# ligengen/EgoGen

Hardware: AMD Instinct MI355X
Metric: PPO env-steps/sec (512 parallel SMPL-X agents) (higher is better)
Workload: dtype f32 (blend GEMM: shape/template columns as 2-term bf16 splits, pose correctives as one fp16 product, fp32 accumulate); PPO update products on 2-term bf16 splits; rollout policy layers on 2-term bf16 splits

## Files before the change

### egogen_amd/_lib.py

```python
from __future__ import annotations

import ctypes as C
import os

_HERE = os.path.dirname(os.path.abspath(__file__))
LIB_PATH = os.path.join(_HERE, "libegogen_hip.so")

c_float_p = C.POINTER(C.c_float)
c_int_p = C.POINTER(C.c_int32)


class EgxError(RuntimeError):
    pass


class BodyModelHost(C.Structure):
    _fields_ = [
        ("num_verts", C.c_int),
        ("v_template_host", C.c_void_p), ("shapedirs_host", C.c_void_p), ("posedirs_host", C.c_void_p),
        ("J_regressor_host", C.c_void_p), ("parents_host", C.c_void_p), ("lbs_weights_host", C.c_void_p),
        ("hand_comps_l_host", C.c_void_p), ("hand_comps_r_host", C.c_void_p),
        ("hand_mean_l_host", C.c_void_p), ("hand_mean_r_host", C.c_void_p),
        ("extra_vids_host", C.c_void_p), ("lmk_vids_host", C.c_void_p), ("lmk_bary_host", C.c_void_p),
        ("num_markers", C.c_int), ("marker_vids_host", C.c_void_p),
# ... 143 lines not shown
    "egx_sample_action": (C.c_int, [C.c_void_p, C.c_void_p, C.c_void_p, C.c_float, C.c_float, C.c_int, C.c_int, C.c_void_p,
                                    C.c_void_p, C.c_void_p]),
    "egx_gae": (C.c_int, [C.c_void_p, C.c_void_p, C.c_void_p, C.c_int, C.c_int, C.c_double, C.c_double, C.c_void_p,
                          C.c_void_p, C.c_void_p]),
    "egx_ppo_loss": (C.c_int, [C.c_void_p] * 9 + [C.c_float] * 6 + [C.c_int] + [C.c_void_p] * 5),
    "egx_gru_pointwise_bwd": (C.c_int, [C.c_void_p, C.c_void_p, C.c_void_p, C.c_void_p, C.c_int, C.c_int, C.c_void_p, C.c_void_p,
                                        C.c_void_p, C.c_void_p]),
    "egx_ppo_loss_packed": (C.c_int, [C.c_void_p] * 8 + [C.c_float] * 6 + [C.c_int] + [C.c_void_p] * 4),
    "egx_lbs_set_blend_mode": (C.c_int, [C.c_int]),
    "egx_lbs_get_blend_mode": (C.c_int, []),
    "egx_lbs_set_wave_tile": (C.c_int, [C.c_int]),
    "egx_lbs_get_wave_tile": (C.c_int, []),
    "egx_lbs_set_fix_queue_capacity": (C.c_int, [C.c_int]),
    "egx_lbs_fix_stats": (C.c_int, [C.c_void_p, C.c_void_p, C.c_int, C.POINTER(C.c_int32)]),
    "egx_gather_rows": (C.c_int, [C.c_void_p, C.c_int, C.c_int, C.c_void_p, C.c_void_p, C.c_void_p, C.c_void_p]),
    "egx_adv_stats": (C.c_int, [C.c_void_p, C.c_int, C.c_void_p, C.c_void_p]),
    "egx_track_episode": (C.c_int, [C.c_void_p, C.c_void_p, C.c_int, C.c_void_p, C.c_void_p, C.c_void_p, C.c_void_p]),
    "egx_rollout_store": (C.c_int, [C.c_void_p] * 6 + [C.c_int] + [C.c_void_p] * 10),
    "egx_adamw_workspace_floats": (C.c_size_t, []),
    "egx_adamw_clip_step": (C.c_int, [C.c_void_p, C.c_void_p, C.c_void_p, C.c_void_p, C.c_size_t, C.c_size_t, C.c_float] + [C.c_double] * 5 +
                            [C.c_void_p, C.c_void_p, C.c_void_p]),
    "egx_policy_set_precision": (C.c_int, [C.c_int]),
    "egx_policy_get_precision": (C.c_int, []),
    "egx_act_fwd": (C.c_int, [C.c_void_p, C.c_void_p, C.c_void_p, C.c_int, C.c_int, C.c_int, C.c_float, C.c_void_p]),
    "egx_act_bwd_colsum": (C.c_int, [C.c_void_p, C.c_void_p, C.c_void_p, C.c_void_p, C.c_int, C.c_int, C.c_int, C.c_float,
                                     C.c_void_p]),
    "egx_profile_next_lbs": (C.c_int, [C.c_void_p, C.c_void_p]),
    "egx_event_create": (C.c_int, [C.POINTER(C.c_void_p)]),
    "egx_event_destroy": (C.c_int, [C.c_void_p]),
    "egx_event_elapsed_ms": (C.c_int, [C.c_void_p, C.c_void_p, C.POINTER(C.c_float)]),
    "egx_policy_train_create": (C.c_int, [C.POINTER(PolicyWeights), C.POINTER(PolicyGrads), C.c_int, C.POINTER(C.c_void_p)]),
    "egx_policy_train_destroy": (None, [C.c_void_p]),
    "egx_policy_train_refresh": (C.c_int, [C.c_void_p, C.c_void_p]),
    "egx_policy_train_packed": (C.c_int, [C.c_void_p, C.POINTER(PolicyPacked3)]),
    "egx_policy_train_bind": (C.c_int, [C.c_void_p, C.c_void_p, C.c_void_p]),
    "egx_policy_train_step": (C.c_int, [C.c_void_p] * 9 + [C.c_float] * 6 + [C.c_void_p, C.c_void_p]),
    "egx_policy_train_step_heads": (C.c_int, [C.c_void_p] * 9 + [C.c_float] * 6 + [C.c_void_p, C.c_void_p]),
    "egx_policy_train_step_encoders": (C.c_int, [C.c_void_p, C.c_void_p]),
    "egx_policy_train_set_precision": (C.c_int, [C.c_void_p, C.c_int]),
    "egx_pack3_bytes": (C.c_size_t, [C.c_int, C.c_int]),
    "egx_pack3": (C.c_int, [C.c_void_p, C.c_int, C.c_int, C.c_int, C.c_int, C.c_void_p, C.c_int, C.c_int, C.c_void_p]),
    "egx_gemm3_workspace_bytes": (C.c_size_t, [C.c_int, C.c_int, C.c_int]),
    "egx_gemm3": (C.c_int, [C.c_void_p, C.c_int, C.c_int, C.c_void_p, C.c_int, C.c_int, C.c_int, C.c_int, C.c_int, C.c_void_p, C.c_int,
                            C.c_float, C.c_void_p, C.c_int, C.c_void_p, C.c_int, C.c_void_p, C.c_int, C.c_void_p, C.c_size_t, C.c_void_p]),
    "egx_vposer_workspace_bytes": (C.c_size_t, [C.c_int]),
    "egx_vposer_encode": (C.c_int, [C.POINTER(VposerWeights), C.c_void_p, C.c_int, C.c_int, C.c_void_p, C.c_void_p,
                                    C.c_size_t, C.c_void_p]),
}

_lib = None


def load():
    global _lib
    if _lib is not None:
        return _lib
    if not os.path.exists(LIB_PATH):
        raise EgxError(f"{LIB_PATH} not found - build it with `python -c 'import __graft_entry__ as g; g.build()'` "
                       f"or `make -C egogen_amd/csrc`; there is no CPU fallback")
    lib = C.CDLL(LIB_PATH)
    for name, (res, args) in SIGNATURES.items():
        fn = getattr(lib, name)
        fn.restype = res
        fn.argtypes = args
    _lib = lib
    return lib


def check(rc: int, what: str):
    if rc != 0:
        msg = load().egx_last_error()
        raise EgxError(f"{what} failed (code {rc}): {msg.decode() if msg else ''}")


def ptr(t):
    if t is None:
        return None
    assert t.is_contiguous(), "tensor must be contiguous"
    return C.c_void_p(t.data_ptr())


def current_stream_ptr():
    import torch
    return C.c_void_p(torch.cuda.current_stream().cuda_stream)
```

### egogen_amd/csrc/egx_nets.h

```cpp
#pragma once
#include "egx_common.h"

struct EgxSeg {
  const float* p;
  int w, ld;
};

int egx_launch_linear(hipStream_t st, int M, int N, const EgxSeg* segs, int nseg, const float* W, const float* b,
                      int act, float slope, const float* res, int ldr, float* out, int ldo);
int egx_launch_gru_pointwise(hipStream_t st, const float* gi, const float* gh, const float* hprev, int ldh, float* hout,
                             int ldo, int M, int H);
int egx_launch_cont6d_to_aa(hipStream_t st, const float* xb6, int n, float* out, int ldo);
int egx_launch_posenc(hipStream_t st, const float* dist, const float* time, int A, float* out);

void egx_launch_frame_scan(hipStream_t st, float* y, const float* x_last, int x_ld, int A, int width, int T);

struct D3Pack {
  const float* src;
  int R, K, ld, col0;
  void* dst;
  int S_total, s0;
  int transpose = 0;
};
void egx_launch_pack3(hipStream_t st, const D3Pack* jobs, int njobs);
// ... 4 lines not shown
  const bf16x8* B = nullptr;
  int S = 0;
  const float* bias = nullptr;
  const float* res = nullptr;
  int ldr = 0;
  float* out = nullptr;
  int ldo = 0;
  bf16x8* out3 = nullptr;
  int S3 = 0, s30 = 0;
  int M = 0, N = 0, act = 0;
  float slope = 0.f;
  int batches = 1;
  size_t batch_strideA = 0, batch_stride3 = 0;
  int batch_rows_out = 0;
  int prec = 0;
  float* out_act = nullptr;
  int ldact = 0;
  const float* dact = nullptr;
  int lddact = 0, dact_code = 0;
  float dact_slope = 0.f;
  bf16x8* out3T = nullptr;
  int S3T = 0, s3T0 = 0;
  float* bias_out = nullptr;
  int n_split = 0;
};
void egx_launch_dense3_n(hipStream_t st, const D3Plain* ps, int n);
void egx_launch_dense3(hipStream_t st, const D3Plain& p);
void egx_launch_dense3_pair(hipStream_t st, const D3Plain& p, const D3Plain& q);
void egx_launch_dense3_triple(hipStream_t st, const D3Plain& p, const D3Plain& q, const D3Plain& r);
int egx_ppo_loss_packed_precleared(const float* zp, const float* value, const float* act, const float* adv, const float* ret,
                                   const float* logp_old, const float* adv_stats, const float* scale, float adv_eps, float min_logvar,
                                   float max_logvar, float eps_clip, float vf_coef, float ent_coef, int num_rows, float* g_zp,
                                   float* g_value, float* out_terms, void* stream_);
void egx_launch_posenc3(hipStream_t st, const float* dist, const float* time, int n, float* out, int ld, void* out3, int S3, int s0,
                        void* out3T = nullptr, int S3T = 0, int col0T = 0, float* zero6 = nullptr );

struct D3Gru {
  const bf16x8* Ai = nullptr;
  int SAi = 0, sai0 = 0;
  const bf16x8* Bi = nullptr;
  int Si = 0;
  const float* bias_i = nullptr;
  const float* gi_in = nullptr;
  float* gi_out = nullptr;
  const bf16x8* Ah = nullptr;
  int SAh = 0, sah0 = 0;
  const bf16x8* Bh = nullptr;
  int Sh = 0;
  const float* bias_h = nullptr;
  const float* h_prev = nullptr;
  int ldh = 0;
  float* h_out = nullptr;
  int ldo = 0;
  bf16x8* h_out3 = nullptr;
  int S3 = 0, s30 = 0;
  int M = 0, H = 0;
  int prec = 0;
  float* gh_out = nullptr;
  bf16x8* h_out3T = nullptr;
  int S3T = 0, s3T0 = 0, col0T = 0;
};
int egx_launch_gru3(hipStream_t st, const D3Gru& g);
int egx_launch_gru3_pair(hipStream_t st, const D3Gru& g0, const D3Gru& g1);

struct RegWeights3 {
  const bf16x8 *in_m, *in_xb, *in_b3;
// ... 36 lines not shown
```

### egogen_amd/csrc/ppo.hip

```cpp
#include <algorithm>
#include <cstring>
#include "egx_common.h"

namespace {
constexpr float LOG_SQRT_2PI = 0.91893853320467274178f;

}

__device__ __forceinline__ float egx_wave_sum(float v) {
#pragma unroll
  for (int o = 32; o > 0; o >>= 1) v += __shfl_xor(v, o);
  return v;
}

__global__ __launch_bounds__(256) void egx_ppo_loss_kernel(const float* __restrict__ mu, const float* __restrict__ logvar,
                                                          const float* __restrict__ value, const float* __restrict__ act,
                                                          const float* __restrict__ adv, const float* __restrict__ ret,
                                                          const float* __restrict__ logp_old, const float* __restrict__ adv_stats,
                                                          const float* __restrict__ scale_ptr, float adv_eps, float min_lv,
                                                          float max_lv, float eps_clip, float vf_coef, float ent_coef, int n,
                                                          int stride ,
                                                          float* __restrict__ g_mu, float* __restrict__ g_logvar,
                                                          float* __restrict__ g_value, float* __restrict__ out_terms) {
  __shared__ float sh[4][6];
// ... 438 lines not shown
}

extern "C" int egx_rollout_store(const float* state, const float* egosensing, const float* dist, const float* time, const float* rew,
                                 const int32_t* term, int num_agents, float* state_dst, float* ego_dst, float* dist_dst, float* time_dst,
                                 float* rew_dst, int32_t* term_dst, float* ep_ret, float* ep_len, float* done_sums, void* stream_) {
  EGX_REQUIRE(state && egosensing && dist && time && state_dst && ego_dst && dist_dst && time_dst && num_agents > 0, "bad arguments");
  EGX_REQUIRE((!rew_dst && !term_dst && !ep_ret) || (rew && term && rew_dst && term_dst), "reward / termination source or slot missing");
  EGX_REQUIRE(!ep_ret || (ep_len && done_sums && rew && term), "episode bookkeeping needs ep_len, done_sums, rew, term");
  hipLaunchKernelGGL(egx_rollout_store_kernel, dim3(num_agents + (ep_ret ? 1 : 0)), dim3(256), 0, static_cast<hipStream_t>(stream_), state,
                     egosensing, dist, time, rew, term, num_agents, state_dst, ego_dst, dist_dst, time_dst, rew_dst, term_dst, ep_ret, ep_len,
                     done_sums);
  EGX_HIP_CHECK(hipGetLastError());
  return EGX_OK;
}

extern "C" size_t egx_adamw_workspace_floats(void) { return 1024 + 8; }

extern "C" int egx_adamw_clip_step(float* param, const float* grad, float* exp_avg, float* exp_avg_sq, size_t n, size_t n_clip,
                                   float max_norm, double lr, double beta1, double beta2, double eps, double weight_decay,
                                   float* step, float* workspace, void* stream_) {
  EGX_REQUIRE(param && grad && exp_avg && exp_avg_sq && step && workspace && n > 0 && n_clip <= n, "bad arguments");
  hipStream_t st = static_cast<hipStream_t>(stream_);
  const int nb = 1024;
  const bool do_clip = max_norm > 0.f && n_clip > 0;
  hipLaunchKernelGGL(egx_sumsq_partial_kernel, dim3(nb), dim3(256), 0, st, grad, do_clip ? n_clip : (size_t)0, workspace, step);
  hipLaunchKernelGGL(egx_adamw_consts_kernel, dim3(1), dim3(256), 0, st, workspace, nb, do_clip ? 1 : 0, max_norm, lr, beta1, beta2,
                     step, workspace + nb);
  const size_t blocks = (n + 1023) / 1024;
  hipLaunchKernelGGL(egx_adamw_flat_kernel, dim3((unsigned)blocks), dim3(256), 0, st, param, grad, exp_avg, exp_avg_sq, n, n_clip,
                     workspace + nb, lr, beta1, beta2, eps, weight_decay);
  EGX_HIP_CHECK(hipGetLastError());
  return EGX_OK;
}
```

### egogen_amd/csrc/update3.hip

```cpp
#include <algorithm>
#include <cstring>
#include <vector>
#include "egx_nets.h"

namespace {

typedef __bf16 bf16v8 __attribute__((ext_vector_type(8)));
__device__ __forceinline__ void u3_split(const float (&x)[8], bf16x8 (&pl)[3]) {
  float r[8];
#pragma unroll
  for (int p = 0; p < 3; ++p) {
    bf16v8 h;
#pragma unroll
    for (int e = 0; e < 8; ++e) {
      const float v = (p == 0) ? x[e] : r[e];
      h[e] = (__bf16)v;
      r[e] = v - (float)h[e];
    }
    pl[p] = __builtin_bit_cast(bf16x8, h);
  }
}

struct PackEntry {
  const float* src;
// ... 56 lines not shown
      bf16x8* o = e.dst2 + ((size_t)(2 * bj + t) * e.S_total2 + bi) * 3 * 64 + lane;
#pragma unroll
      for (int p = 0; p < 3; ++p)
        if (p < nplanes) o[p * 64] = pl[p];
    }
    return;
  }
  if (!e.transpose) {
    const int S = (e.cols + 31) >> 5;
    rt = frag / S; s = frag % S;
    const int row = rt * 16 + (lane & 15), k0 = s * 32 + 8 * (lane >> 4);
#pragma unroll
    for (int q = 0; q < 8; ++q) x[q] = (row < e.red && k0 + q < e.cols) ? e.src[(size_t)row * e.ld + e.col0 + k0 + q] : 0.f;
  } else {
    const int S = (e.red + 31) >> 5;
    rt = frag / S; s = frag % S;
    const int irow = rt * 16 + (lane & 15), k0 = s * 32 + 8 * (lane >> 4);
#pragma unroll
    for (int q = 0; q < 8; ++q) {
      float v = 0.f;
      if (k0 + q < e.red) {
        if (irow < e.cols) v = e.src[(size_t)(k0 + q) * e.ld + e.col0 + irow];
        else if (irow == e.ones_row) v = 1.f;
      }
      x[q] = v;
    }
  }
  bf16x8 pl[3];
  u3_split(x, pl);
  bf16x8* o = e.dst + ((size_t)rt * e.S_total + e.s0 + s) * 3 * 64 + lane;
#pragma unroll
  for (int p = 0; p < 3; ++p)
    if (p < nplanes) o[p * 64] = pl[p];
}

inline int img_tiles(int rows) { return 2 * egx_ceil_div(rows, 32); }
inline size_t img_frags(int rows, int red) { return (size_t)img_tiles(rows) * egx_ceil_div(red, 32); }
constexpr size_t FRAG_BYTES = 3 * 64 * 16;

struct GruBwd {
  const float* gi;
  const float* gh;
  const float* bias_h;
  const float* h_prev;
  const float* dh0;
  const float* dh1;
  int ld0, ld1;
  bf16x8* dgiT;
  bf16x8* dghT;
  int ST, s0T;
  bf16x8* dgh_r;
  float* dhp;
  int M, H;
};
struct GruBwd2 {
  GruBwd a, b;
  int blocks0;
};

__global__ __launch_bounds__(256) void egx_gru_bwd3_kernel(GruBwd2 two) {
  const bool second = (int)blockIdx.x >= two.blocks0;
  const GruBwd& a = second ? two.b : two.a;
  const int bid = second ? (int)blockIdx.x - two.blocks0 : (int)blockIdx.x;
  __shared__ __attribute__((aligned(16))) float tile[6][32 * 36];
  const int CT = a.H >> 5;
  const int mt = bid / CT, ct = bid % CT;
// ... 72 lines not shown
  bf16x8 *a1_r, *u1_r, *a3_r, *u2_r, *a1T, *u1T, *a3T, *u2T;
  bf16x8 *g_r[4], *gT[4];
  float* head;
  float* ghead;
  bf16x8 *ghead_r, *gheadT;
};
struct Encoder {
  const float *Wih, *Whh, *bih, *bhh;
  float *gWih, *gWhh, *gbih, *gbhh;
  int in_dim, cat_off;
  bf16x8 *Wih_r, *Whh_r, *Whh_t;
  bf16x8 *x0_r, *x1_r, *xT;
  float *gi1, *gi2, *gh2, *h1f;
  bf16x8 *h1_r, *hprevT;
  bf16x8 *dgiT, *dghT, *dgh_r;
  float *dhp, *dh1;
};

}

struct egx_policy_train {
  int n = 0, Sn = 0;
  Arena ar;
  Encoder enc[2];
  Branch br[2];
  float* catf = nullptr;
  bf16x8 *cat_r = nullptr, *catT = nullptr;
  PackEntry* tab_weights = nullptr; int n_weights = 0, frags_weights = 0;
  PackEntry* tab_inputs = nullptr; int n_inputs = 0, frags_inputs = 0;
  PackEntry* tab_loss = nullptr; int n_loss = 0, frags_loss = 0;
  std::vector<PackEntry> h_inputs;
  const float* bound_state = nullptr; const float* bound_ego = nullptr;
  int prec = 0;
};

namespace {

int upload_table(std::vector<PackEntry>& v, PackEntry** dev, int* frags) {
  int run = 0;
  for (PackEntry& e : v) {
    if (e.transpose == 2) {
      run += egx_ceil_div(e.red, 32) * egx_ceil_div(e.cols, 32);
    } else {
      const int rows = e.transpose ? e.cols + (e.ones_row >= 0 ? 1 : 0) : e.red;
      const int red = e.transpose ? e.red : e.cols;
      run += (int)img_frags(rows, red);
    }
    e.frag_end = run;
  }
  *frags = run;
  if (!*dev) EGX_HIP_CHECK(hipMalloc(reinterpret_cast<void**>(dev), v.size() * sizeof(PackEntry)));
  EGX_HIP_CHECK(hipMemcpy(*dev, v.data(), v.size() * sizeof(PackEntry), hipMemcpyHostToDevice));
  return EGX_OK;
}
void run_table(hipStream_t st, const PackEntry* tab, int n, int frags, int nplanes = 3) {
  hipLaunchKernelGGL(egx_pack3_table_kernel, dim3(egx_ceil_div(frags, 4)), dim3(256), 0, st, tab, n, nplanes);
}
inline int planes_of(int prec) { return prec == 0 ? 3 : (prec == 2 ? 2 : 1); }

void layout(egx_policy_train* h) {
  const int n = h->n, Sn = h->Sn;
  Arena& ar = h->ar;
  ar.off = 0;
  auto img = [&](int rows, int red) { return static_cast<bf16x8*>(ar.take(img_frags(rows, red) * FRAG_BYTES)); };
  auto f32 = [&](size_t count) { return static_cast<float*>(ar.take(count * sizeof(float))); };
  for (int e = 0; e < 2; ++e) {
// ... 72 lines not shown
  ones(h->catT, CAT, Sn, 0, Sn);
  for (int b = 0; b < 2; ++b)
    for (bf16x8* img : {h->br[b].a1T, h->br[b].u1T, h->br[b].a3T, h->br[b].u2T}) ones(img, CAT, Sn, 0, Sn);
  U3_CHECK(hipGetLastError());
  std::vector<PackEntry> tw;
  auto add = [](std::vector<PackEntry>& v, const float* src, int red, int cols, int ld, int col0, bf16x8* dst, int S_total, int s0,
                int transpose, int ones_row) {
    PackEntry e;
    e.src = src; e.red = red; e.cols = cols; e.ld = ld; e.col0 = col0; e.dst = dst; e.S_total = S_total; e.s0 = s0;
    e.transpose = transpose; e.ones_row = ones_row; e.frag_end = 0; e.dst2 = nullptr; e.S_total2 = 0;
    v.push_back(e);
  };
  auto add_both = [](std::vector<PackEntry>& v, const float* src, int rows, int cols, bf16x8* img, bf16x8* imgT) {
    PackEntry e;
    e.src = src; e.red = rows; e.cols = cols; e.ld = cols; e.col0 = 0; e.dst = img; e.S_total = egx_ceil_div(cols, 32); e.s0 = 0;
    e.transpose = 2; e.ones_row = -1; e.frag_end = 0; e.dst2 = imgT; e.S_total2 = egx_ceil_div(rows, 32);
    v.push_back(e);
  };
  for (int e = 0; e < 2; ++e) {
    Encoder& En = h->enc[e];
    add(tw, En.Wih, 3 * HD, En.in_dim, En.in_dim, 0, En.Wih_r, egx_ceil_div(En.in_dim, 32), 0, 0, -1);
    add_both(tw, En.Whh, 3 * HD, HD, En.Whh_r, En.Whh_t);
  }
  for (int b = 0; b < 2; ++b) {
    Branch& B = h->br[b];
    for (int l = 0; l < 4; ++l) {
      add_both(tw, B.W[l], CAT, CAT, B.W_r[l], B.W_t[l]);
    }
    add_both(tw, B.Wout, B.nout, CAT, B.Wout_r, B.Wout_t);
  }
  h->n_weights = (int)tw.size();
  int rc = upload_table(tw, &h->tab_weights, &h->frags_weights);
  if (rc) return fail(rc);
  for (int e = 0; e < 2; ++e) {
    Encoder& En = h->enc[e];
    const int d = En.in_dim, S = egx_ceil_div(d, 32);
    add(h->h_inputs, nullptr, n, d, 2 * d, 0, En.x0_r, S, 0, 0, -1);
    add(h->h_inputs, nullptr, n, d, 2 * d, d, En.x1_r, S, 0, 0, -1);
    add(h->h_inputs, nullptr, n, d, 2 * d, 0, En.xT, 2 * Sn, 0, 1, d);
    add(h->h_inputs, nullptr, n, d, 2 * d, d, En.xT, 2 * Sn, Sn, 1, d);
  }
  h->n_inputs = (int)h->h_inputs.size();
  std::vector<PackEntry> tl;
  for (int b = 0; b < 2; ++b) {
    Branch& B = h->br[b];
    add(tl, B.ghead, n, B.nout, B.nout, 0, B.ghead_r, egx_ceil_div(B.nout, 32), 0, 0, -1);
    add(tl, B.ghead, n, B.nout, B.nout, 0, B.gheadT, Sn, 0, 1, -1);
  }
  h->n_loss = (int)tl.size();
  if ((rc = upload_table(tl, &h->tab_loss, &h->frags_loss))) return fail(rc);
  U3_CHECK(hipDeviceSynchronize());
#undef U3_CHECK
  *out = h;
  return EGX_OK;
}

extern "C" void egx_policy_train_destroy(egx_policy_train* h) {
  if (!h) return;
  (void)hipFree(h->ar.base); (void)hipFree(h->tab_weights); (void)hipFree(h->tab_inputs); (void)hipFree(h->tab_loss);
  delete h;
}

extern "C" int egx_policy_train_refresh(egx_policy_train* h, void* stream) {
  EGX_REQUIRE(h, "null handle");
  const int planes = std::max(planes_of(h->prec), planes_of(egx_policy_get_precision()));
  run_table(static_cast<hipStream_t>(stream), h->tab_weights, h->n_weights, h->frags_weights, planes);
  EGX_HIP_CHECK(hipGetLastError());
  return EGX_OK;
}

extern "C" int egx_policy_train_set_precision(egx_policy_train* h, int prec) {
  EGX_REQUIRE(h, "null handle");
  EGX_REQUIRE(prec == 0 || prec == 1 || prec == 2, "precision must be 0 (three bf16 planes: fp32-equivalent), 2 (two planes) or 1 (bf16)");
  h->prec = prec;
  return EGX_OK;
}

extern "C" int egx_policy_train_packed(const egx_policy_train* h, egx_policy_packed3* out) {
  EGX_REQUIRE(h && out, "null argument");
  out->x_enc_w_ih = h->enc[0].Wih_r; out->x_enc_w_hh = h->enc[0].Whh_r;
  out->ego_enc_w_ih = h->enc[1].Wih_r; out->ego_enc_w_hh = h->enc[1].Whh_r;
  for (int l = 0; l < 4; ++l) { out->actor_w[l] = h->br[0].W_r[l]; out->critic_w[l] = h->br[1].W_r[l]; }
  out->actor_out_w = h->br[0].Wout_r; out->critic_out_w = h->br[1].Wout_r;
  return EGX_OK;
}

extern "C" int egx_policy_train_bind(egx_policy_train* h, const float* state, const float* egosensing) {
  EGX_REQUIRE(h && state && egosensing, "null argument");
  if (h->bound_state == state && h->bound_ego == egosensing && h->tab_inputs) return EGX_OK;
  for (int i = 0; i < 4; ++i) h->h_inputs[i].src = state;
  for (int i = 4; i < 8; ++i) h->h_inputs[i].src = egosensing;
  int rc = upload_table(h->h_inputs, &h->tab_inputs, &h->frags_inputs);
  if (rc) return rc;
  h->bound_state = state; h->bound_ego = egosensing;
  return EGX_OK;
}

static int train_step_parts(egx_policy_train* h, const float* dist, const float* time, const float* act, const float* adv,
                            const float* ret, const float* logp_old, const float* adv_stats, const float* scale, float adv_eps,
// ... 209 lines not shown
```

### egogen_amd/ppo_policy.py

```python
from __future__ import annotations

import ctypes as C
import math
import os
from typing import Dict, List, Optional

import numpy as np
import torch
import torch.distributed as dist
from torch import nn

from . import _lib
from .models import ActorCritic, GAMMAActor, GAMMACritic, GAMMAPolicyBase, PolicyHipRunner

_EPS = float(np.finfo(np.float32).eps)
_LOG_SQRT_2PI = math.log(math.sqrt(2 * math.pi))
_UPDATE_PREC = {"f32": 0, "bf16x2": 2, "bf16": 1}


class RunningMeanStd:

    def __init__(self):
        self.mean, self.var, self.count = 0.0, 1.0, 0

# ... 53 lines not shown
        self._value_clip = bool(value_clip)
        self._rew_norm = bool(reward_normalization)
        self._recompute_adv = bool(recompute_advantage)
        self.ret_rms = RunningMeanStd()
        self.actor, self.critic, self.shared_net = actor, critic, shared_net
        self._actor_critic = ActorCritic(actor, critic)
        self.optim = optim
        self._gamma, self._lambda = discount_factor, gae_lambda
        self._grad_norm = max_grad_norm
        self._weight_vf, self._weight_ent, self._weight_kld = vf_coef, ent_coef, weight_kld
        self._eps_clip = eps_clip
        self._norm_adv = bool(advantage_normalization)
        self._deterministic_eval = deterministic_eval
        self._batch = max_batchsize
        self._runner = PolicyHipRunner(shared_net, actor, critic)
        self._noise_gen: Optional[torch.Generator] = None
        self._seed = seed
        self._perm_gen = torch.Generator().manual_seed(seed)
        self._flat_grad: Optional[torch.Tensor] = None
        self._after_minibatch = None
        self._layout = None
        self._graph_cache: dict = {}
        self.use_update_graph = bool(_ignored.get("use_update_graph", False))
        self.overlap_allreduce = os.environ.get("EGX_DP_OVERLAP", "0") == "1"
        self.use_fused_loss = bool(_ignored.get("use_fused_loss", True))
        self._scale_cache = {}
        self.use_train_step = bool(_ignored.get("use_train_step", os.environ.get("EGX_TRAIN_STEP", "1") != "0"))
        self._train_handles: dict = {}
        self.update_precision = str(_ignored.get("update_precision", os.environ.get("EGX_UPDATE_PREC", "f32")))
        if self.update_precision not in _UPDATE_PREC:
            raise ValueError(f"update_precision must be one of {sorted(_UPDATE_PREC)}, got {self.update_precision!r}")
        self.use_fused_linear = bool(_ignored.get("use_fused_linear", True))
        self.use_flat_optimizer = bool(_ignored.get("use_flat_optimizer", os.environ.get("EGX_FLAT_OPTIMIZER", "1") != "0"))
        self._flat_opt_state = None
        self.world_size = dist.get_world_size() if dist.is_available() and dist.is_initialized() else 1
        self._dp = self.world_size > 1 or (os.environ.get("EGX_FORCE_DP_PATH") == "1" and dist.is_available() and dist.is_initialized())
        self.update_paths: dict = {}
        self.allreduce_events: list = []
        self._allreduce_done: list = []

    @torch.no_grad()
    def forward(self, obs: Dict[str, torch.Tensor], noise: Optional[torch.Tensor] = None, out: Optional[dict] = None):
        lib = _lib.load()
        out = self._runner.forward(obs, want_actor=True, want_critic=True, out=out)
        n = out["mu"].shape[0]
        dev = out["mu"].device
        deterministic = self._deterministic_eval and not self.training
        if not deterministic and noise is None:
            if self._noise_gen is None:
                self._noise_gen = torch.Generator(device=dev)
                rank = dist.get_rank() if self.world_size > 1 else 0
                self._noise_gen.manual_seed(self._seed + 1 + 9973 * rank)
            noise = torch.randn(n, 128, generator=self._noise_gen, device=dev)
        if "act" not in out:
            out["act"] = torch.empty(n, 128, dtype=torch.float32, device=dev)
            out["logp"] = torch.empty(n, dtype=torch.float32, device=dev)
        rc = lib.egx_sample_action(_lib.ptr(out["mu"]), _lib.ptr(out["logvar"]), _lib.ptr(noise) if noise is not None else None,
                                   float(self.actor.min_logvar), float(self.actor.max_logvar), 1 if deterministic else 0, n,
                                   _lib.ptr(out["act"]), _lib.ptr(out["logp"]), _lib.current_stream_ptr())
        _lib.check(rc, "egx_sample_action")
        return out

    @torch.no_grad()
    def values(self, obs: Dict[str, torch.Tensor]) -> torch.Tensor:
        return self._runner.forward(obs, want_actor=False, want_critic=True)["value"]

# ... 128 lines not shown
            return hs
        if self._graph_cache:
            self._graph_cache.clear()
        lib = _lib.load()
        self._ensure_flat_grads()
        w = self._runner._weights()
        g = _lib.PolicyGrads()
        s, a, c = self.shared_net, self.actor.pnet, self.critic.vnet
        gp = lambda t: t.grad.data_ptr()
        g.x_enc_w_ih, g.x_enc_w_hh, g.x_enc_b_ih, g.x_enc_b_hh = gp(s.x_enc.weight_ih_l0), gp(s.x_enc.weight_hh_l0), gp(s.x_enc.bias_ih_l0), gp(s.x_enc.bias_hh_l0)
        g.ego_enc_w_ih, g.ego_enc_w_hh, g.ego_enc_b_ih, g.ego_enc_b_hh = (gp(s.ego_enc.weight_ih_l0), gp(s.ego_enc.weight_hh_l0),
                                                                            gp(s.ego_enc.bias_ih_l0), gp(s.ego_enc.bias_hh_l0))
        for b in range(2):
            for k in range(2):
                g.actor_w[2 * b + k], g.actor_b[2 * b + k] = gp(a.layers[b].layers[k].weight), gp(a.layers[b].layers[k].bias)
                g.critic_w[2 * b + k], g.critic_b[2 * b + k] = gp(c.layers[b].layers[k].weight), gp(c.layers[b].layers[k].bias)
        g.actor_out_w, g.actor_out_b = gp(a.out_fc.weight), gp(a.out_fc.bias)
        g.critic_out_w, g.critic_out_b = gp(c.out_fc.weight), gp(c.out_fc.bias)
        h = C.c_void_p()
        _lib.check(lib.egx_policy_train_create(C.byref(w), C.byref(g), int(n), C.byref(h)), "egx_policy_train_create")
        _lib.check(lib.egx_policy_train_set_precision(h, _UPDATE_PREC[self.update_precision]), "egx_policy_train_set_precision")
        dev = self._flat_grad.device
        f = dict(dtype=torch.float32, device=dev)
        bufs = [torch.empty(n, 804, **f), torch.empty(n, 64, **f), torch.empty(n, 1, **f), torch.empty(n, 1, **f),
                torch.empty(n, 128, **f), torch.empty(n, 1, **f), torch.empty(n, 1, **f), torch.empty(n, 1, **f)]
        _lib.check(lib.egx_policy_train_bind(h, _lib.ptr(bufs[0]), _lib.ptr(bufs[1])), "egx_policy_train_bind")
        packed = _lib.PolicyPacked3()
        _lib.check(lib.egx_policy_train_packed(h, C.byref(packed)), "egx_policy_train_packed")
        hs = {"h": h, "bufs": bufs, "stats": torch.zeros(2, **f), "key": (w.x_enc_w_ih, g.x_enc_w_ih), "packed": packed}
        self._train_handles[n] = hs
        if len(self._train_handles) == 1:
            self._runner.adopt_packed(packed, refresh=self._refresh_images)
            self._images_owner = n
        self._refresh_images()
        return hs

    def _chain_shapes_ok(self) -> bool:
        ok = getattr(self, "_chain_ok", None)
        if ok is None:
            a, c, s = self.actor.pnet, self.critic.vnet, self.shared_net
            def block_ok(blk, nout):
                return (blk.residual and len(blk.layers) == 2 and blk.out_fc.out_features == nout and blk.out_fc.in_features == 1152
                        and all(m.act_name == "lrelu" and len(m.layers) == 2 and
                                all(fc.in_features == 1152 and fc.out_features == 1152 for fc in m.layers) for m in blk.layers))
            ok = (s.h_dim == 512 and s.x_enc.input_size == 402 and s.ego_enc.input_size == 32 and block_ok(a, 256) and block_ok(c, 1))
            self._chain_ok = ok
        return ok

    def _drop_train_handles(self):
        lib = _lib.load() if self._train_handles else None
        for hs in self._train_handles.values():
            lib.egx_policy_train_destroy(hs["h"])
        self._train_handles = {}
        self._runner._wstruct = None

    def __del__(self):
        try:
            self._drop_train_handles()
        except Exception:
            pass

    def _refresh_images(self):
        if not self._train_handles:
            return
        lib, st = _lib.load(), _lib.current_stream_ptr()
        for hs in self._train_handles.values():
            _lib.check(lib.egx_policy_train_refresh(hs["h"], st), "egx_policy_train_refresh")

    def _fwd_bwd_train_step(self, hs, batch, idx, gstats, log_out, part: str = "all"):
        from .fused_ops import gather_rows
        lib, st = _lib.load(), _lib.current_stream_ptr()
        if part == "encoders":
            _lib.check(lib.egx_policy_train_step_encoders(hs["h"], st), "egx_policy_train_step_encoders")
            return
        N = batch.n * batch.A
        obs_all = batch.obs_flat()
        b = hs["bufs"]
        gather_rows(idx, [obs_all["state"].reshape(N, 804), obs_all["egosensing"].reshape(N, 64), obs_all["dist"].reshape(N, 1),
                          obs_all["time"].reshape(N, 1), batch.act.reshape(N, 128), batch.adv.reshape(N, 1), batch.returns.reshape(N, 1),
                          batch.logp_old.reshape(N, 1)], out=b)
        n = int(idx.shape[0])
        dev = b[0].device
        if gstats is None:
            _lib.check(lib.egx_adv_stats(_lib.ptr(b[5]), n, _lib.ptr(hs["stats"]), st), "egx_adv_stats")
            scale = self._scale_cache.get((n, dev))
            if scale is None:
                scale = torch.full((1,), 1.0 / n, dtype=torch.float32, device=dev)
                self._scale_cache[(n, dev)] = scale
        else:
            hs["stats"].copy_(torch.stack([gstats[0], gstats[1]]).float())
            scale = (1.0 / gstats[2]).reshape(1).float()
        fn = lib.egx_policy_train_step_heads if part == "heads" else lib.egx_policy_train_step
        rc = fn(hs["h"], _lib.ptr(b[2]), _lib.ptr(b[3]), _lib.ptr(b[4]), _lib.ptr(b[5]), _lib.ptr(b[6]), _lib.ptr(b[7]),
                _lib.ptr(hs["stats"]), _lib.ptr(scale), float(_EPS), float(self.actor.min_logvar),
                float(self.actor.max_logvar), float(self._eps_clip), float(self._weight_vf), float(self._weight_ent),
                _lib.ptr(log_out), st)
        _lib.check(rc, "egx_policy_train_step")

    def _fwd_bwd(self, batch, idx, gstats, log_out) -> str:
        hs = self._train_handle(int(idx.shape[0])) if idx.is_cuda else None
        if hs is not None:
            self._fwd_bwd_train_step(hs, batch, idx, gstats, log_out)
            return "chain"
        obs, act, adv, ret, lpo = self._gather(batch, idx)
        v_s = batch.values[:batch.n].reshape(-1).index_select(0, idx) if self._value_clip else None
        loss, terms = self.minibatch_loss(obs, act, adv, ret, lpo, gstats, v_s=v_s)
        self._flat_grad.zero_()
        loss.backward()
        if adv.is_cuda and self.use_fused_loss and self.use_fused_linear:
            from . import models as _m
            if _m._TWO_STREAM_UPDATE:
                torch.cuda.current_stream().wait_stream(_m._side_stream(adv.device))
        packed = terms.get("_packed")
        if packed is not None:
            log_out.copy_(packed)
        else:
            log_out.copy_(torch.stack([terms[k].detach() for k in ("loss", "loss/clip", "loss/vf", "loss/ent", "loss/kld", "approx_kl")]))
        return "autograd"

    def _clip_and_step(self):
        if self.use_flat_optimizer and self._flat_opt_state == "ready":
            g = self.optim.param_groups[0]
            lib = _lib.load()
            b1, b2 = g["betas"]
            rc = lib.egx_adamw_clip_step(_lib.ptr(self._flat_p), _lib.ptr(self._flat_grad), _lib.ptr(self._flat_m), _lib.ptr(self._flat_v),
                                         self._flat_p.numel(), self._n_clip, float(self._grad_norm or 0.0), float(g["lr"]), float(b1),
                                         float(b2), float(g["eps"]), float(g["weight_decay"]), _lib.ptr(self._step_t),
                                         _lib.ptr(self._adamw_ws), _lib.current_stream_ptr())
            _lib.check(rc, "egx_adamw_clip_step")
            self._runner.mark_dirty()
            self._refresh_images()
            return
        if self._grad_norm:
            nn.utils.clip_grad_norm_(self._actor_critic.parameters(), max_norm=self._grad_norm)
        self.optim.step()
        self._refresh_images()

    def _flat_optimizer_ready(self) -> bool:
        if self._flat_opt_state == "unsupported":
            return False
        opt = self.optim
        params = [p for g in opt.param_groups for p in g["params"]]
        if self._flat_opt_state is None:
            ok = (isinstance(opt, torch.optim.AdamW) and len(opt.param_groups) == 1 and not opt.param_groups[0].get("amsgrad", False)
                  and not opt.param_groups[0].get("maximize", False) and all(p.is_cuda and p.dtype == torch.float32 for p in params))
            clip = list(self._actor_critic.parameters())
            ok = ok and len(clip) <= len(params) and all(a is b for a, b in zip(clip, params))
            if not ok:
                self._flat_opt_state = "unsupported"
                return False
            dev = params[0].device
            lay = self._flat_layout()
            total = self._layout_total
            self._flat_p = torch.zeros(total, dtype=torch.float32, device=dev)
            self._flat_m = torch.zeros(total, dtype=torch.float32, device=dev)
            self._flat_v = torch.zeros(total, dtype=torch.float32, device=dev)
            self._step_t = torch.zeros((), dtype=torch.float32, device=dev)
            self._adamw_ws = torch.zeros(int(_lib.load().egx_adamw_workspace_floats()), dtype=torch.float32, device=dev)
            self._n_clip = lay[len(clip)][1] if len(clip) < len(lay) else total
            with torch.no_grad():
                for p, off, n in lay:
                    self._flat_p[off:off + n].copy_(p.detach().reshape(-1))
                    p.data = self._flat_p[off:off + n].view_as(p)
            self._flat_opt_state = "ready"
# ... 271 lines not shown
```

### include/egogen_hip.h

```cpp
#ifndef EGOGEN_HIP_H
#define EGOGEN_HIP_H

#include <stddef.h>
#include <stdint.h>

#ifdef __cplusplus
extern "C" {
#endif

#define EGX_OK 0
#define EGX_ERR_ARG (-1)
#define EGX_ERR_HIP (-2)
#define EGX_ERR_WORKSPACE (-3)

#define EGX_NUM_JOINTS 55
#define EGX_NUM_JOINTS_OUT 127
#define EGX_XB_DIM 93
#define EGX_NUM_BETAS 10
#define EGX_POSE_FEAT 486
#define EGX_BLEND_K 472

const char* egx_last_error(void);
int egx_version(void);

typedef struct egx_body_model egx_body_model;

typedef struct egx_body_model_host {
  int num_verts;
  const float* v_template_host;
  const float* shapedirs_host;
  const float* posedirs_host;
  const float* J_regressor_host;
  const int32_t* parents_host;
  const float* lbs_weights_host;
  const float* hand_comps_l_host;
  const float* hand_comps_r_host;
  const float* hand_mean_l_host;
  const float* hand_mean_r_host;
  const int32_t* extra_vids_host;
  const int32_t* lmk_vids_host;
  const float* lmk_bary_host;
  int num_markers;
  const int32_t* marker_vids_host;
  int num_feet;
  const int32_t* feet_vids_host;
} egx_body_model_host;
// ... 139 lines not shown
size_t egx_sample_prior_workspace_bytes(int num_agents);

int egx_sample_prior(const egx_prior_weights* w, const float* x_hist0, const float* x_hist1, int x_ld,
                     const float* betas, const float* z, int num_agents, float* out_Y, float* out_Yb,
                     void* workspace, size_t workspace_bytes, void* stream);

typedef struct egx_policy_packed3 {
  const void *x_enc_w_ih, *x_enc_w_hh;
  const void *ego_enc_w_ih, *ego_enc_w_hh;
  const void *actor_w[4], *actor_out_w;
  const void *critic_w[4], *critic_out_w;
} egx_policy_packed3;

typedef struct egx_policy_weights {
  const float *x_enc_w_ih, *x_enc_w_hh, *x_enc_b_ih, *x_enc_b_hh;
  const float *ego_enc_w_ih, *ego_enc_w_hh, *ego_enc_b_ih, *ego_enc_b_hh;
  const float *actor_w[4], *actor_b[4];
  const float *actor_out_w, *actor_out_b;
  const float *critic_w[4], *critic_b[4];
  const float *critic_out_w, *critic_out_b;
  const egx_policy_packed3* packed3;
} egx_policy_weights;

typedef struct egx_policy_grads {
  float *x_enc_w_ih, *x_enc_w_hh, *x_enc_b_ih, *x_enc_b_hh;
  float *ego_enc_w_ih, *ego_enc_w_hh, *ego_enc_b_ih, *ego_enc_b_hh;
  float *actor_w[4], *actor_b[4], *actor_out_w, *actor_out_b;
  float *critic_w[4], *critic_b[4], *critic_out_w, *critic_out_b;
} egx_policy_grads;
typedef struct egx_policy_train egx_policy_train;
int egx_policy_train_create(const egx_policy_weights* w, const egx_policy_grads* g, int num_rows, egx_policy_train** out);
void egx_policy_train_destroy(egx_policy_train* h);
int egx_policy_train_refresh(egx_policy_train* h, void* stream);
int egx_policy_train_packed(const egx_policy_train* h, egx_policy_packed3* out);
int egx_policy_train_bind(egx_policy_train* h, const float* state, const float* egosensing);
int egx_policy_train_step(egx_policy_train* h, const float* dist, const float* time, const float* act, const float* adv,
                          const float* ret, const float* logp_old, const float* adv_stats, const float* scale, float adv_eps,
                          float min_logvar, float max_logvar, float eps_clip, float vf_coef, float ent_coef, float* out_terms,
                          void* stream);
int egx_policy_train_step_heads(egx_policy_train* h, const float* dist, const float* time, const float* act, const float* adv,
                                const float* ret, const float* logp_old, const float* adv_stats, const float* scale, float adv_eps,
                                float min_logvar, float max_logvar, float eps_clip, float vf_coef, float ent_coef, float* out_terms,
                                void* stream);
int egx_policy_train_step_encoders(egx_policy_train* h, void* stream);
int egx_policy_train_set_precision(egx_policy_train* h, int prec);

int egx_policy_set_precision(int bf16);
int egx_policy_get_precision(void);

size_t egx_policy_workspace_bytes(int num_rows);

int egx_policy_forward(const egx_policy_weights* w, const float* state, const float* egosensing, const float* dist,
                       const float* time, int num_rows, float* out_mu, float* out_logvar, float* out_value,
                       void* workspace, size_t workspace_bytes, void* stream);

typedef struct egx_vposer_weights {
  const float *fc1_w, *fc1_b;
  const float *fc2_w, *fc2_b;
  const float *mu_w, *mu_b;
  const void *fc1_w3, *fc2_w3, *mu_w3;
} egx_vposer_weights;

size_t egx_vposer_workspace_bytes(int num_rows);
int egx_vposer_encode(const egx_vposer_weights* w, const float* x, int x_ld, int num_rows, float* out,
                      void* workspace, size_t workspace_bytes, void* stream);

// ... 143 lines not shown
```

Before: 186,000.

## Fuse AdamW step with bf16 weight-image repacking in one kernel

After: 184,800. No clear change (-0.7%).

```diff
diff --git a/egogen_amd/_lib.py b/egogen_amd/_lib.py
--- a/egogen_amd/_lib.py
+++ b/egogen_amd/_lib.py
@@ -199,6 +199,9 @@
     "egx_policy_train_create": (C.c_int, [C.POINTER(PolicyWeights), C.POINTER(PolicyGrads), C.c_int, C.POINTER(C.c_void_p)]),
     "egx_policy_train_destroy": (None, [C.c_void_p]),
     "egx_policy_train_refresh": (C.c_int, [C.c_void_p, C.c_void_p]),
+    "egx_policy_train_bind_flat": (C.c_int, [C.c_void_p, C.c_void_p, C.c_size_t]),
+    "egx_policy_train_adamw_step": (C.c_int, [C.c_void_p] * 5 + [C.c_size_t, C.c_size_t, C.c_float] + [C.c_double] * 5 +
+                                    [C.c_void_p, C.c_void_p, C.c_void_p]),
     "egx_policy_train_packed": (C.c_int, [C.c_void_p, C.POINTER(PolicyPacked3)]),
     "egx_policy_train_bind": (C.c_int, [C.c_void_p, C.c_void_p, C.c_void_p]),
     "egx_policy_train_step": (C.c_int, [C.c_void_p] * 9 + [C.c_float] * 6 + [C.c_void_p, C.c_void_p]),
@@ -234,6 +237,9 @@
     return lib
 
 
+EGX_ERR_LAYOUT = -4
+
+
 def check(rc: int, what: str):
     if rc != 0:
         msg = load().egx_last_error()
diff --git a/egogen_amd/csrc/egx_nets.h b/egogen_amd/csrc/egx_nets.h
--- a/egogen_amd/csrc/egx_nets.h
+++ b/egogen_amd/csrc/egx_nets.h
@@ -60,6 +60,8 @@
                                    const float* logp_old, const float* adv_stats, const float* scale, float adv_eps, float min_logvar,
                                    float max_logvar, float eps_clip, float vf_coef, float ent_coef, int num_rows, float* g_zp,
                                    float* g_value, float* out_terms, void* stream_);
+void egx_launch_adamw_consts(hipStream_t st, const float* grad, size_t n_clip, float max_norm, double lr, double beta1, double beta2,
+                             float* step, float* workspace);
 void egx_launch_posenc3(hipStream_t st, const float* dist, const float* time, int n, float* out, int ld, void* out3, int S3, int s0,
                         void* out3T = nullptr, int S3T = 0, int col0T = 0, float* zero6 = nullptr );
 
diff --git a/egogen_amd/csrc/ppo.hip b/egogen_amd/csrc/ppo.hip
--- a/egogen_amd/csrc/ppo.hip
+++ b/egogen_amd/csrc/ppo.hip
@@ -494,3 +494,12 @@
   EGX_HIP_CHECK(hipGetLastError());
   return EGX_OK;
 }
+
+void egx_launch_adamw_consts(hipStream_t st, const float* grad, size_t n_clip, float max_norm, double lr, double beta1, double beta2,
+                             float* step, float* workspace) {
+  const int nb = 1024;
+  const bool do_clip = max_norm > 0.f && n_clip > 0;
+  hipLaunchKernelGGL(egx_sumsq_partial_kernel, dim3(nb), dim3(256), 0, st, grad, do_clip ? n_clip : (size_t)0, workspace, step);
+  hipLaunchKernelGGL(egx_adamw_consts_kernel, dim3(1), dim3(256), 0, st, workspace, nb, do_clip ? 1 : 0, max_norm, lr, beta1, beta2,
+                     step, workspace + nb);
+}
diff --git a/egogen_amd/csrc/update3.hip b/egogen_amd/csrc/update3.hip
--- a/egogen_amd/csrc/update3.hip
+++ b/egogen_amd/csrc/update3.hip
@@ -112,6 +112,167 @@
 #pragma unroll
   for (int p = 0; p < 3; ++p)
     if (p < nplanes) o[p * 64] = pl[p];
+}
+
+struct AdamArgs {
+  float* p; const float* g; float* m; float* v;
+  size_t n_clip;
+  const float* consts;
+  double lr, b1, b2, eps, wd;
+};
+struct AdamRange {
+  size_t begin, end;
+  int block_end;
+  int pad;
+};
+struct AdamK {
+  float coef, step_size, bc2s;
+  double omb1, omb2, lrwd, b2, eps;
+};
+__device__ __forceinline__ AdamK u3_adamw_consts(const AdamArgs& a) {
+  AdamK k;
+  k.coef = a.consts[0]; k.step_size = a.consts[1]; k.bc2s = a.consts[2];
+  k.omb1 = 1.0 - a.b1; k.omb2 = 1.0 - a.b2; k.lrwd = a.lr * a.wd; k.b2 = a.b2; k.eps = a.eps;
+  return k;
+}
+__device__ __forceinline__ void u3_adamw_elem(float& p, float g, float& m, float& v, bool clip, const AdamK& k) {
+#pragma clang fp contract(off)
+  const float gg = clip ? g * k.coef : g;
+  const double gd = (double)gg, md = (double)m, pd = (double)p;
+  const float pw = (float)__builtin_fma(-k.lrwd, pd, pd);
+  m = (float)__builtin_fma(k.omb1, gd - md, md);
+  v = (float)__builtin_fma(k.omb2 * gd, gd, k.b2 * (double)v);
+  const float denom = (float)((double)(sqrtf(v) / k.bc2s) + k.eps);
+  p = pw - k.step_size * m / denom;
+}
+struct AdamLane8 { float p[8], g[8], m[8], v[8]; };
+__device__ __forceinline__ void u3_adamw_load8(const AdamArgs& a, size_t idx, int nv, AdamLane8& L) {
+  if (nv == 8 && (idx & 3) == 0) {
+    const f32x4 p0 = *reinterpret_cast<const f32x4*>(a.p + idx), p1 = *reinterpret_cast<const f32x4*>(a.p + idx + 4);
+    const f32x4 g0 = *reinterpret_cast<const f32x4*>(a.g + idx), g1 = *reinterpret_cast<const f32x4*>(a.g + idx + 4);
+    const f32x4 m0 = *reinterpret_cast<const f32x4*>(a.m + idx), m1 = *reinterpret_cast<const f32x4*>(a.m + idx + 4);
+    const f32x4 v0 = *reinterpret_cast<const f32x4*>(a.v + idx), v1 = *reinterpret_cast<const f32x4*>(a.v + idx + 4);
+#pragma unroll
+    for (int q = 0; q < 4; ++q) {
+      L.p[q] = p0[q]; L.p[q + 4] = p1[q]; L.g[q] = g0[q]; L.g[q + 4] = g1[q];
+      L.m[q] = m0[q]; L.m[q + 4] = m1[q]; L.v[q] = v0[q]; L.v[q + 4] = v1[q];
+    }
+  } else {
+#pragma unroll
+    for (int q = 0; q < 8; ++q) {
+      const bool in = q < nv;
+      L.p[q] = in ? a.p[idx + q] : 0.f; L.g[q] = in ? a.g[idx + q] : 0.f;
+      L.m[q] = in ? a.m[idx + q] : 0.f; L.v[q] = in ? a.v[idx + q] : 0.f;
+    }
+  }
+}
+__device__ __forceinline__ void u3_adamw_step8(const AdamArgs& a, const AdamK& k, size_t idx, int nv, AdamLane8& L) {
+#pragma unroll
+  for (int q = 0; q < 8; ++q)
+    if (q < nv) u3_adamw_elem(L.p[q], L.g[q], L.m[q], L.v[q], idx + q < a.n_clip, k);
+}
+__device__ __forceinline__ void u3_adamw_store8(const AdamArgs& a, size_t idx, int nv, const AdamLane8& L) {
+  if (nv == 8 && (idx & 3) == 0) {
+    f32x4 p0, p1, m0, m1, v0, v1;
+#pragma unroll
+    for (int q = 0; q < 4; ++q) {
+      p0[q] = L.p[q]; p1[q] = L.p[q + 4]; m0[q] = L.m[q]; m1[q] = L.m[q + 4]; v0[q] = L.v[q]; v1[q] = L.v[q + 4];
+    }
+    *reinterpret_cast<f32x4*>(a.p + idx) = p0; *reinterpret_cast<f32x4*>(a.p + idx + 4) = p1;
+    *reinterpret_cast<f32x4*>(a.m + idx) = m0; *reinterpret_cast<f32x4*>(a.m + idx + 4) = m1;
+    *reinterpret_cast<f32x4*>(a.v + idx) = v0; *reinterpret_cast<f32x4*>(a.v + idx + 4) = v1;
+  } else {
+#pragma unroll
+    for (int q = 0; q < 8; ++q)
+      if (q < nv) { a.p[idx + q] = L.p[q]; a.m[idx + q] = L.m[q]; a.v[idx + q] = L.v[q]; }
+  }
+}
+__device__ __forceinline__ void u3_store_planes(bf16x8* o, const float (&x)[8], int nplanes) {
+  bf16x8 pl[3];
+  u3_split(x, pl);
+#pragma unroll
+  for (int p = 0; p < 3; ++p)
+    if (p < nplanes) o[p * 64] = pl[p];
+}
+
+__global__ __launch_bounds__(256) void egx_adamw_images_kernel(const PackEntry* __restrict__ tab, int n, int nplanes, int frag_blocks,
+                                                               const AdamRange* __restrict__ ranges, int n_ranges, AdamArgs a) {
+  __shared__ float sblk[4][32][33];
+  const AdamK k = u3_adamw_consts(a);
+  if ((int)blockIdx.x >= frag_blocks) {
+    const int b = (int)blockIdx.x - frag_blocks;
+    int ri = 0;
+    while (ri < n_ranges && b >= ranges[ri].block_end) ++ri;
+    if (ri >= n_ranges) return;
+    const AdamRange r = ranges[ri];
+    const size_t i0 = r.begin + ((size_t)(b - (ri > 0 ? ranges[ri - 1].block_end : 0)) * 256 + threadIdx.x) * 4;
+#pragma unroll
+    for (int q = 0; q < 4; ++q) {
+      const size_t i = i0 + q;
+      if (i < r.end) {
+        float pv = a.p[i], mv = a.m[i], vv = a.v[i];
+        u3_adamw_elem(pv, a.g[i], mv, vv, i < a.n_clip, k);
+        a.p[i] = pv; a.m[i] = mv; a.v[i] = vv;
+      }
+    }
+    return;
+  }
+  int frag = blockIdx.x * 4 + (threadIdx.x >> 6);
+  const int lane = threadIdx.x & 63;
+  if (n <= 0 || frag >= tab[n - 1].frag_end) return;
+  int lo = 0, hi = n - 1;
+  while (lo < hi) {
+    const int mid = (lo + hi) >> 1;
+    if (frag >= tab[mid].frag_end) lo = mid + 1; else hi = mid;
+  }
+  const PackEntry e = tab[lo];
+  frag -= lo > 0 ? tab[lo - 1].frag_end : 0;
+  const size_t base = (size_t)(e.src - a.p) + e.col0;
+  const int r = lane & 15, kg = lane >> 4;
+  float x[8];
+  if (e.transpose == 2) {
+    float (*sb)[33] = sblk[threadIdx.x >> 6];
+    const int BJ = (e.cols + 31) >> 5;
+    const int bi = frag / BJ, bj = frag % BJ;
+    const int k0 = 32 * bj + 8 * kg;
+    AdamLane8 L[2];
+    size_t idx[2];
+    int nv[2];
+#pragma unroll
+    for (int t = 0; t < 2; ++t) {
+      const int row = 32 * bi + 16 * t + r;
+      idx[t] = base + (size_t)row * e.ld + k0;
+      nv[t] = row < e.red ? min(max(e.cols - k0, 0), 8) : 0;
+      u3_adamw_load8(a, idx[t], nv[t], L[t]);
+    }
+#pragma unroll
+    for (int t = 0; t < 2; ++t) u3_adamw_step8(a, k, idx[t], nv[t], L[t]);
+#pragma unroll
+    for (int t = 0; t < 2; ++t) {
+      u3_adamw_store8(a, idx[t], nv[t], L[t]);
+#pragma unroll
+      for (int q = 0; q < 8; ++q) sb[16 * t + r][8 * kg + q] = L[t].p[q];
+      u3_store_planes(e.dst + ((size_t)(2 * bi + t) * e.S_total + e.s0 + bj) * 3 * 64 + lane, L[t].p, nplanes);
+    }
+    __builtin_amdgcn_wave_barrier();
+#pragma unroll
+    for (int t = 0; t < 2; ++t) {
+#pragma unroll
+      for (int q = 0; q < 8; ++q) x[q] = sb[8 * kg + q][16 * t + r];
+      u3_store_planes(e.dst2 + ((size_t)(2 * bj + t) * e.S_total2 + bi) * 3 * 64 + lane, x, nplanes);
+    }
+    return;
+  }
+  const int S = (e.cols + 31) >> 5;
+  const int rt = frag / S, s = frag % S;
+  const int row = rt * 16 + r, k0 = s * 32 + 8 * kg;
+  const size_t idx = base + (size_t)row * e.ld + k0;
+  const int nv = row < e.red ? min(max(e.cols - k0, 0), 8) : 0;
+  AdamLane8 L;
+  u3_adamw_load8(a, idx, nv, L);
+  u3_adamw_step8(a, k, idx, nv, L);
+  u3_adamw_store8(a, idx, nv, L);
+  u3_store_planes(e.dst + ((size_t)rt * e.S_total + e.s0 + s) * 3 * 64 + lane, L.p, nplanes);
 }
 
 inline int img_tiles(int rows) { return 2 * egx_ceil_div(rows, 32); }
@@ -250,6 +411,9 @@
   std::vector<PackEntry> h_inputs;
   const float* bound_state = nullptr; const float* bound_ego = nullptr;
   int prec = 0;
+  std::vector<PackEntry> h_weights;
+  const float* flat_p = nullptr; size_t flat_n = 0;
+  AdamRange* adam_ranges = nullptr; int n_adam_ranges = 0, adam_range_blocks = 0;
 };
 
 namespace {
@@ -388,6 +552,7 @@
   h->n_weights = (int)tw.size();
   int rc = upload_table(tw, &h->tab_weights, &h->frags_weights);
   if (rc) return fail(rc);
+  h->h_weights = tw;
   for (int e = 0; e < 2; ++e) {
     Encoder& En = h->enc[e];
     const int d = En.in_dim, S = egx_ceil_div(d, 32);
@@ -414,6 +579,7 @@
 extern "C" void egx_policy_train_destroy(egx_policy_train* h) {
   if (!h) return;
   (void)hipFree(h->ar.base); (void)hipFree(h->tab_weights); (void)hipFree(h->tab_inputs); (void)hipFree(h->tab_loss);
+  (void)hipFree(h->adam_ranges);
   delete h;
 }
 
@@ -421,6 +587,71 @@
   EGX_REQUIRE(h, "null handle");
   const int planes = std::max(planes_of(h->prec), planes_of(egx_policy_get_precision()));
   run_table(static_cast<hipStream_t>(stream), h->tab_weights, h->n_weights, h->frags_weights, planes);
+  EGX_HIP_CHECK(hipGetLastError());
+  return EGX_OK;
+}
+
+extern "C" int egx_policy_train_bind_flat(egx_policy_train* h, const float* flat_param, size_t n) {
+  EGX_REQUIRE(h && flat_param && n > 0, "bad arguments");
+  h->flat_p = nullptr; h->flat_n = 0;
+  std::vector<std::pair<size_t, size_t>> runs;
+  for (const PackEntry& e : h->h_weights) {
+    const size_t len = (size_t)e.red * e.ld;
+    if ((e.transpose != 0 && e.transpose != 2) || e.col0 != 0 || e.ld != e.cols || e.src < flat_param ||
+        (size_t)(e.src - flat_param) + len > n) {
+      egx_set_error("egx_policy_train_bind_flat: a weight matrix lies outside the flat parameter buffer");
+      return EGX_ERR_LAYOUT;
+    }
+    runs.emplace_back((size_t)(e.src - flat_param), (size_t)(e.src - flat_param) + len);
+  }
+  std::sort(runs.begin(), runs.end());
+  std::vector<AdamRange> comp;
+  size_t at = 0;
+  int blocks = 0;
+  auto gap = [&](size_t b, size_t e_) {
+    if (e_ <= b) return;
+    blocks += (int)((e_ - b + 1023) / 1024);
+    comp.push_back(AdamRange{b, e_, blocks, 0});
+  };
+  for (const auto& r : runs) {
+    if (r.first < at) {
+      egx_set_error("egx_policy_train_bind_flat: weight matrices overlap in the flat parameter buffer");
+      return EGX_ERR_LAYOUT;
+    }
+    gap(at, r.first);
+    at = r.second;
+  }
+  gap(at, n);
+  if (comp.size() > (size_t)h->n_adam_ranges || !h->adam_ranges) {
+    (void)hipFree(h->adam_ranges);
+    h->adam_ranges = nullptr;
+    EGX_HIP_CHECK(hipMalloc(reinterpret_cast<void**>(&h->adam_ranges), std::max<size_t>(comp.size(), 1) * sizeof(AdamRange)));
+  }
+  if (!comp.empty()) EGX_HIP_CHECK(hipMemcpy(h->adam_ranges, comp.data(), comp.size() * sizeof(AdamRange), hipMemcpyHostToDevice));
+  h->n_adam_ranges = (int)comp.size(); h->adam_range_blocks = blocks;
+  h->flat_p = flat_param; h->flat_n = n;
+  return EGX_OK;
+}
+
+extern "C" int egx_policy_train_adamw_step(egx_policy_train* h, float* param, const float* grad, float* exp_avg, float* exp_avg_sq,
+                                           size_t n, size_t n_clip, float max_norm, double lr, double beta1, double beta2, double eps,
+                                           double weight_decay, float* step, float* workspace, void* stream) {
+  EGX_REQUIRE(h && param && grad && exp_avg && exp_avg_sq && step && workspace && n > 0 && n_clip <= n, "bad arguments");
+  EGX_REQUIRE(((reinterpret_cast<uintptr_t>(param) | reinterpret_cast<uintptr_t>(grad) | reinterpret_cast<uintptr_t>(exp_avg) |
+                reinterpret_cast<uintptr_t>(exp_avg_sq)) & 15) == 0, "the flat buffers must be 16-byte aligned");
+  if (!h->flat_p || h->flat_p != param || h->flat_n != n) {
+    egx_set_error("egx_policy_train_adamw_step: the handle is not bound to this flat parameter buffer (egx_policy_train_bind_flat)");
+    return EGX_ERR_LAYOUT;
+  }
+  hipStream_t st = static_cast<hipStream_t>(stream);
+  egx_launch_adamw_consts(st, grad, n_clip, max_norm, lr, beta1, beta2, step, workspace);
+  const int planes = std::max(planes_of(h->prec), planes_of(egx_policy_get_precision()));
+  const int frag_blocks = egx_ceil_div(h->frags_weights, 4);
+  AdamArgs a;
+  a.p = param; a.g = grad; a.m = exp_avg; a.v = exp_avg_sq; a.n_clip = n_clip; a.consts = workspace + 1024;
+  a.lr = lr; a.b1 = beta1; a.b2 = beta2; a.eps = eps; a.wd = weight_decay;
+  hipLaunchKernelGGL(egx_adamw_images_kernel, dim3(frag_blocks + h->adam_range_blocks), dim3(256), 0, st, h->tab_weights, h->n_weights,
+                     planes, frag_blocks, h->adam_ranges, h->n_adam_ranges, a);
   EGX_HIP_CHECK(hipGetLastError());
   return EGX_OK;
 }
diff --git a/egogen_amd/ppo_policy.py b/egogen_amd/ppo_policy.py
--- a/egogen_amd/ppo_policy.py
+++ b/egogen_amd/ppo_policy.py
@@ -109,6 +109,9 @@
             raise ValueError(f"update_precision must be one of {sorted(_UPDATE_PREC)}, got {self.update_precision!r}")
         self.use_fused_linear = bool(_ignored.get("use_fused_linear", True))
         self.use_flat_optimizer = bool(_ignored.get("use_flat_optimizer", os.environ.get("EGX_FLAT_OPTIMIZER", "1") != "0"))
+        self.use_fused_adamw = bool(_ignored.get("use_fused_adamw", os.environ.get("EGX_FUSED_ADAMW", "1") != "0"))
+        self.image_refreshes = 0
+        self.fused_adamw_steps = 0
         self._flat_opt_state = None
         self.world_size = dist.get_world_size() if dist.is_available() and dist.is_initialized() else 1
         self._dp = self.world_size > 1 or (os.environ.get("EGX_FORCE_DP_PATH") == "1" and dist.is_available() and dist.is_initialized())
@@ -303,6 +306,12 @@
         if len(self._train_handles) == 1:
             self._runner.adopt_packed(packed, refresh=self._refresh_images)
             self._images_owner = n
+            hs["fused_adamw"] = False
+            if self.use_fused_adamw:
+                rc = lib.egx_policy_train_bind_flat(h, _lib.ptr(self._flat_p), self._flat_p.numel())
+                if rc != _lib.EGX_ERR_LAYOUT:
+                    _lib.check(rc, "egx_policy_train_bind_flat")
+                    hs["fused_adamw"] = True
         self._refresh_images()
         return hs
 
@@ -331,12 +340,15 @@
         except Exception:
             pass
 
-    def _refresh_images(self):
+    def _refresh_images(self, skip=None):
         if not self._train_handles:
             return
         lib, st = _lib.load(), _lib.current_stream_ptr()
         for hs in self._train_handles.values():
+            if hs is skip:
+                continue
             _lib.check(lib.egx_policy_train_refresh(hs["h"], st), "egx_policy_train_refresh")
+            self.image_refreshes += 1
 
     def _fwd_bwd_train_step(self, hs, batch, idx, gstats, log_out, part: str = "all"):
         from .fused_ops import gather_rows
@@ -394,13 +406,19 @@
             g = self.optim.param_groups[0]
             lib = _lib.load()
             b1, b2 = g["betas"]
-            rc = lib.egx_adamw_clip_step(_lib.ptr(self._flat_p), _lib.ptr(self._flat_grad), _lib.ptr(self._flat_m), _lib.ptr(self._flat_v),
-                                         self._flat_p.numel(), self._n_clip, float(self._grad_norm or 0.0), float(g["lr"]), float(b1),
-                                         float(b2), float(g["eps"]), float(g["weight_decay"]), _lib.ptr(self._step_t),
-                                         _lib.ptr(self._adamw_ws), _lib.current_stream_ptr())
-            _lib.check(rc, "egx_adamw_clip_step")
+            args = (_lib.ptr(self._flat_p), _lib.ptr(self._flat_grad), _lib.ptr(self._flat_m), _lib.ptr(self._flat_v),
+                    self._flat_p.numel(), self._n_clip, float(self._grad_norm or 0.0), float(g["lr"]), float(b1),
+                    float(b2), float(g["eps"]), float(g["weight_decay"]), _lib.ptr(self._step_t),
+                    _lib.ptr(self._adamw_ws), _lib.current_stream_ptr())
+            owner = self._train_handles.get(getattr(self, "_images_owner", None))
+            if owner is not None and owner.get("fused_adamw"):
+                _lib.check(lib.egx_policy_train_adamw_step(owner["h"], *args), "egx_policy_train_adamw_step")
+                self.fused_adamw_steps += 1
+            else:
+                owner = None
+                _lib.check(lib.egx_adamw_clip_step(*args), "egx_adamw_clip_step")
             self._runner.mark_dirty()
-            self._refresh_images()
+            self._refresh_images(skip=owner)
             return
         if self._grad_norm:
             nn.utils.clip_grad_norm_(self._actor_critic.parameters(), max_norm=self._grad_norm)
diff --git a/include/egogen_hip.h b/include/egogen_hip.h
--- a/include/egogen_hip.h
+++ b/include/egogen_hip.h
@@ -12,6 +12,7 @@
 #define EGX_ERR_ARG (-1)
 #define EGX_ERR_HIP (-2)
 #define EGX_ERR_WORKSPACE (-3)
+#define EGX_ERR_LAYOUT (-4)
 
 #define EGX_NUM_JOINTS 55
 #define EGX_NUM_JOINTS_OUT 127
@@ -217,6 +218,10 @@
 int egx_policy_train_create(const egx_policy_weights* w, const egx_policy_grads* g, int num_rows, egx_policy_train** out);
 void egx_policy_train_destroy(egx_policy_train* h);
 int egx_policy_train_refresh(egx_policy_train* h, void* stream);
+int egx_policy_train_bind_flat(egx_policy_train* h, const float* flat_param, size_t n);
+int egx_policy_train_adamw_step(egx_policy_train* h, float* param, const float* grad, float* exp_avg, float* exp_avg_sq, size_t n,
+                                size_t n_clip, float max_norm, double lr, double beta1, double beta2, double eps,
+                                double weight_decay, float* step, float* workspace, void* stream);
 int egx_policy_train_packed(const egx_policy_train* h, egx_policy_packed3* out);
 int egx_policy_train_bind(egx_policy_train* h, const float* state, const float* egosensing);
 int egx_policy_train_step(egx_policy_train* h, const float* dist, const float* time, const float* act, const float* adv,
```
